# OpenRobotLab/EmbodiedScan

Measured on AMD Instinct MI355X. Metric: scans/sec (train step) mv-3ddet, 20x(480x640) RGB-D views, higher is better.
Workload: dtype bf16; 1 GPU; mv-3ddet ResNet-50(w16) + MinkResNet34 + FCAF3DHeadRotMat, 20 views 480x640, 100k points/scan, bf16 matrix cores with f32 accumulate / f32 master weights, full train step incl. H2D of the batch and AdamW; views=20, parallelism=dp1, h2d=157 MB per step as ONE copy from a pinned slab on a copy stream, double-buffered

## Files before the change

embodiedscan_amd/csrc/imgconv.hip:

```cpp
#include "common.h"
#include "../../include/es_hip.h"

typedef float f32x4 __attribute__((ext_vector_type(4)));
typedef __bf16 bf16x8_t __attribute__((ext_vector_type(8)));

__device__ __attribute__((aligned(16))) unsigned short g_ic_zero[8];

template <int C, int WP, int S, int MODE>
__global__ __launch_bounds__(256) void k_img_conv3(const void* __restrict__ Xv, int ldx, const unsigned short* __restrict__ Wt,
                                                   const float* __restrict__ scale, const float* __restrict__ shift,
                                                   const unsigned short* __restrict__ gate, int ldg, void* __restrict__ Yv, int ldy,
                                                   int y_half, int act, int H, int W, int rows_per_wg, int bands) {
  static_assert(MODE == 0 || S == 1, "the gated data gradient is built for stride 1");
  constexpr int RB = C * 2;
  constexpr int XP = S * WP + 2, X_BYTES = XP * RB;
  constexpr int NS = S == 1 ? 4 : 8;
  constexpr int GX = RB / 16;
  constexpr int NCB = C / 16;
  constexpr bool CO_SPLIT = NCB >= 4;
  constexpr int CBW = CO_SPLIT ? NCB / 4 : NCB;
  constexpr bool PAIR = C == 16;
  constexpr int KS = PAIR ? 1 : C / 32;
  constexpr int NT = PAIR ? 5 : 9;
  constexpr int NPB = WP / 16;
// ... 124 lines not shown
            }
          } else if (px < Wo) {
            const float gt = __uint_as_float((uint32_t)gate[row * ldg + col] << 16);
            ((float*)Yv)[row * ldy + col] = gt > 0.f ? v : 0.f;
          }
        }
      }
    }
  }
}

static int ES_OPT_IMG_CONV = 1;
static int ES_OPT_IMG_CONV_WGS = 1024;
extern "C" int es_img_conv_set_option(int key, int value) {
  if (key == 50) { ES_OPT_IMG_CONV = value; return 0; }
  if (key == 51) { ES_OPT_IMG_CONV_WGS = value; return 0; }
  return -1;
}

static bool img_conv_plan(int n_img, int H, int W, int C, int stride, int mode, int& wp, int& rows, int& bands) {
  if (!ES_OPT_IMG_CONV || n_img <= 0 || H <= 0 || W <= 0) return false;
  if (mode == 1 && stride != 1) return false;
  if (stride != 1 && !(stride == 2 && H % 2 == 0 && W % 2 == 0)) return false;
  const int Ho = H / stride, Wo = W / stride;
  if (C == 16 && Wo <= 128 && stride == 1) wp = Wo <= 64 ? 64 : 128;
  else if (C == 32 && Wo <= 64) wp = 64;
  else if (C == 64 && Wo <= 32) wp = 32;
  else return false;
  if (C == 64 && stride == 2) return false;
  const int target = (C == 64 || stride == 2) ? ES_OPT_IMG_CONV_WGS / 2 : ES_OPT_IMG_CONV_WGS;
  bands = target / n_img;
  if (bands < 1) bands = 1;
  if (bands > Ho) bands = Ho;
  rows = es_cdiv(Ho, bands);
  bands = es_cdiv(Ho, rows);
  return true;
}

static bool img_conv_check(int n_img, int H, int W, int C, int stride, int mode, const void* X, int ldx, const void* W_bf16,
                           const void* Y, int y_half, int ldy, int& wp, int& rows, int& bands) {
  if (!img_conv_plan(n_img, H, W, C, stride, mode, wp, rows, bands)) return false;
  if ((ldx % (mode ? 4 : 8)) || ((((uintptr_t)X) | ((uintptr_t)W_bf16)) & 15) || (y_half ? ((ldy % 2) || (((uintptr_t)Y) & 3)) : 0)) return false;
  if (mode == 1 && y_half) return false;
  return (long long)n_img * H * W * (ldx > ldy ? ldx : ldy) < (1ll << 31);
}

extern "C" int es_img_conv3_supported(int n_img, int H, int W, int C, int stride, int mode) {
  int wp, rows, bands;
  return img_conv_check(n_img, H, W, C, stride, mode, nullptr, C, nullptr, nullptr, 0, C, wp, rows, bands) ? 1 : 0;
}

extern "C" int es_img_conv3_bf16(const void* X, int ldx, const void* W_bf16, int n_img, int H, int W, int C, int stride, int mode,
                                 const float* scale, const float* shift, const void* gate, int ldg, int act, void* Y, int y_half,
                                 int ldy, void* stream) {
  int wp, rows, bands;
  if (!img_conv_check(n_img, H, W, C, stride, mode, X, ldx, W_bf16, Y, y_half, ldy, wp, rows, bands)) return -4;
  if (mode == 1 && gate == nullptr) return -4;
  if (mode == 0 && act != 0 && act != 1) return -4;
  hipStream_t st = (hipStream_t)stream;
  const unsigned short* Wt = (const unsigned short*)W_bf16;
  const unsigned short* G = (const unsigned short*)gate;
#define IC_LAUNCH(C_, WP_, S_, M_)                                                                                           \
  hipLaunchKernelGGL((k_img_conv3<C_, WP_, S_, M_>), dim3(n_img * bands), dim3(256), 0, st, X, ldx, Wt, scale, shift, G, ldg, Y, ldy, \
                     y_half, act, H, W, rows, bands)
  if (mode == 0 && stride == 1) {
    if (C == 16 && wp == 128) IC_LAUNCH(16, 128, 1, 0);
    else if (C == 16) IC_LAUNCH(16, 64, 1, 0);
    else if (C == 32) IC_LAUNCH(32, 64, 1, 0);
    else IC_LAUNCH(64, 32, 1, 0);
  } else if (mode == 0) {
    if (C == 32) IC_LAUNCH(32, 64, 2, 0);
    else if (C == 64) IC_LAUNCH(64, 32, 2, 0);
    else return -4;
  } else {
    if (C == 16 && wp == 128) IC_LAUNCH(16, 128, 1, 1);
    else if (C == 16) IC_LAUNCH(16, 64, 1, 1);
    else if (C == 32) IC_LAUNCH(32, 64, 1, 1);
    else IC_LAUNCH(64, 32, 1, 1);
  }
#undef IC_LAUNCH
  ES_CHECK_LAUNCH();
  return 0;
}
```

embodiedscan_amd/engine.py:

```python
import os

import torch
from . import hip
from .hip import P, call, iarr


def _stream():
    return hip.stream()


_NEW_VARS = None


class Var:
    __slots__ = ('d', 'g', 'rg', 'dh', 'gh', 'gate', 'gated', 'fresh')

    def __init__(self, d, rg=True):
        self.d, self.g, self.rg = d, None, rg
        self.dh = self.gh = None
        if _NEW_VARS is not None:
            _NEW_VARS.append(self)
        self.fresh = False
        self.gate = None
        self.gated = False
# ... 241 lines not shown
    ws['used'] = True
    _KEEP.extend(keep)
    return ws['h']


def wgrad_stream_obj():
    return _wgrad_rec()['s']


def join_wgrad_streams(final=True):
    cur = hip.stream_obj()
    for ws in _WGRAD_STREAMS.values():
        if ws['used']:
            ws['join'].record(ws['s'])
            cur.wait_event(ws['join'])
            ws['used'] = False
    if final:
        _KEEP.clear()


_ZEROED = ('ticket', 'split', 'colsum', 'topk')
_WS = {tag: {} for tag in ('wgrad', 'dense') + _ZEROED}
_WGRAD_WS = _WS['wgrad']


def stream_ws(stream, tag, floats, like):
    table = _WS[tag]
    ws = table.get(stream)
    if ws is None or ws.numel() < floats or ws.device != like.device:
        if ws is not None:
            _KEEP.append(ws)
        if tag in _ZEROED:
            ws = torch.zeros(max(int(floats), 1 << 16), dtype=torch.float32, device=like.device)
            if stream != _stream():
                ev = torch.cuda.Event()
                ev.record(hip.stream_obj())
                hip._stream_of(stream).wait_event(ev)
        else:
            ws = torch.empty(max(int(floats), 1 << 22), dtype=torch.float32, device=like.device)
        table[stream] = ws
    return ws, ws.numel()


def ticket_ws(floats, like, tag='ticket'):
    assert tag in _ZEROED, tag
    return stream_ws(_stream(), tag, floats, like)


GRAD_EPOCH = [1]
_GRAD_STAMP = {}


def new_grad_epoch():
    GRAD_EPOCH[0] += 1
    if len(_GRAD_STAMP) > 1 << 16:
        _GRAD_STAMP.clear()


def _first_write(ptr):
    acc = 1 if _GRAD_STAMP.get(ptr) == GRAD_EPOCH[0] else 0
    _GRAD_STAMP[ptr] = GRAD_EPOCH[0]
    return acc


def _written(ptr):
    return 1 if _GRAD_STAMP.get(ptr) == GRAD_EPOCH[0] else 0


def _wgrad(name, sw, dW, *args, like=None, acc=None):
    if name == 'es_spconv_wgrad_bf16_src':
        X, xh, ldx, dY, yh, ldy, nbr, n_out, n_in, K, cin, cout = args
        need = hip.raw('es_spconv_wgrad_workspace_floats')(1, X, xh, ldx, dY, yh, ldy, n_out, n_in, K, cin, cout)
    else:
        X, ldx, dY, ldy, nbr, n_out, n_in, K, cin, cout = args
        need = hip.raw('es_spconv_wgrad_workspace_floats')(int(name == 'es_spconv_wgrad_bf16'), X, 0, ldx, dY, 0, ldy, n_out, n_in,
                                                           K, cin, cout)
    if like is None:
        like = torch.empty(0, device=torch.device('cuda', torch.cuda.current_device()))
    ws, nf = stream_ws(sw, 'wgrad', need, like) if need else (None, 0)
    call(name, *args, dW, _first_write(dW) if acc is None else acc, P(ws), nf, sw)


IMG_WGRAD = [os.environ.get('ES_IMG_WGRAD', '1') != '0']
HEAD_BWD_FUSED = [os.environ.get('ES_HEAD_BWD_FUSED', '1') != '0']


GC_SETTLE_STEP = 6


_HOST_SETTLED = [False]


def settle_host_threads(force=False):
    if _HOST_SETTLED[0] and not force:
        return
    _HOST_SETTLED[0] = True
    want = os.environ.get('ES_HOST_THREADS', 'auto')
    if want == '0':
        return
    if want == 'auto':
        from .datasets.loader import effective_cpus
        local = max(1, int(os.environ.get('LOCAL_WORLD_SIZE', '1') or 1))
        n = max(1, effective_cpus() // 4 // local)
    else:
        n = max(1, int(want))
    if torch.get_num_threads() > n:
        torch.set_num_threads(n)


def settle_gc(det):
    settle_host_threads()
    n = getattr(det, '_steps_done', 0) + 1
    det._steps_done = n
    if n == GC_SETTLE_STEP and os.environ.get('ES_GC_FREEZE', '1') != '0':
        import gc
        gc.collect()
        gc.freeze()
        _GC_FROZEN[0] = True


def reset_tickets():
    for tag in _ZEROED:
        for ws in _WS[tag].values():
            ws[:min(ws.numel(), 2048)].zero_()


def drop_caches():
    for table in _WS.values():
        table.clear()
    _KEEP.clear()


MARKS = None


HOST_MARKS = None


def mark(name):
    if HOST_MARKS is not None:
        import time
        HOST_MARKS.append((name, time.perf_counter()))
    if MARKS is not None:
        ev = torch.cuda.Event(enable_timing=True)
        ev.record(hip.stream_obj())
        MARKS.append((name, ev))


DEBUG_GRADS = None
DEBUG_CONV = None
DEBUG_OPS = None
DEBUG_FWD = None


def fwd_record(kind, entry, **ops):
    rec = dict(kind=kind, entry=entry, precision=PRECISION[0])
    for k, v in ops.items():
        if isinstance(v, (Param, ParamSlice)):
            rec[k] = v.d.clone()
            if PRECISION[0] == 'bf16' and v.d.dim() == 3:
                rec[k + '_h'] = v.bf16()[1].clone()
        elif isinstance(v, torch.Tensor):
            rec[k] = v.clone()
        else:
            rec[k] = v
    if callable(DEBUG_FWD):
# ... 183 lines not shown
    x.fresh = False
    y.fresh = True
    return y


def _conv_backward(x, w, nbr, inv, n_out, y, gy, bias, bias_from, need_dx, bf, gate=None, dense=None, maps=None, img=None):
    K, cin, cout = w.d.shape
    rec = None
    dn_ok = bf and dense is not None and gate is None and _ld(gy) == cout and _ld(x.d) == cin
    dn_w = dense if (dn_ok and w.g is not None and dense_ok(dense, 2, cin, cout)) else None
    dn_d = dense if (dn_ok and need_dx and x.rg and dense_ok(dense, 1, cin, cout)) else None
    if maps is not None and (DEBUG_CONV is not None or (w.g is not None and dn_w is None) or (need_dx and x.rg and dn_d is None)):
        nbr, inv = maps.get()
    if DEBUG_CONV is not None:
        rec = dict(x=x.d, w=w, nbr=nbr, n_out=n_out, gy=gy.clone(), bf=bool(bf), gate=gate, need_dx=bool(need_dx and x.rg),
                   before=(x.g.clone() if (x.g is not None and need_dx and x.rg) else None), bias=bias, bias_from=bias_from)
        DEBUG_CONV.append(rec)
    gh = None
    if dn_w is not None or dn_d is not None or (
            bf and cout >= 16 and need_dx and x.rg and gate is None and _ld(gy) == cout and _use_shadow(n_out, cout, K, cout, cin)):
        gh = y.grad_shadow() if gy is y.g else _cast_rows(gy)
    if dn_w is not None:
        x.shadow()
    if w.g is not None or (bias is not None and bias.g is not None):
        sw = _wgrad_stream(gy, x.d, gh, x.dh)
    if w.g is not None:
        _conv_wgrad(x, w, nbr, n_out, gy, gh, bf, dn_w, maps, img, sw)
    if bias is not None and bias.g is not None:
        nb, dst = cout - bias_from, bias.g.data_ptr() + 4 * bias_from
        ws, nf = stream_ws(sw, 'colsum', int(hip.raw('es_colsum_workspace_floats')(n_out, nb)), gy)
        call('es_colsum', gy.data_ptr() + 4 * bias_from, _ld(gy), n_out, nb, dst, _first_write(dst), P(ws), nf, sw)
    if need_dx and x.rg:
        _conv_dgrad(x, w, inv, n_out, gy, gh, bf, dn_d, maps, gate, img)
    if rec is not None and rec['need_dx']:
        rec['after'] = x.g.clone()


def _conv_wgrad(x, w, nbr, n_out, gy, gh, bf, dn_w, maps, img, sw):
    K, cin, cout = w.d.shape
    n_in = x.d.shape[0]
    acc = _first_write(P(w.g))
    xh_f32 = bf and x.dh is not None and gy.dtype == torch.float32
    if dn_w is not None:
        if _dense_wgrad(P(x.dh), cin, P(gh), cout, dn_w, 0, cin, cout, P(w.g), acc, sw, gh):
            return
        if maps is not None:
            nbr, _ = maps.get()
            sw = _wgrad_stream()
    if IMG_WGRAD[0] and xh_f32 and img is not None and K == 9 and cin == cout:
        nf = int(hip.raw('es_img_wgrad9_workspace_floats')(img[0], img[1], img[2], cin, img[3]))
        if nf:
            ws, nf = stream_ws(sw, 'wgrad', nf, gy)
            if hip.try_call('es_img_wgrad9_bf16', P(x.dh), _ld(x.dh), P(gy), _ld(gy), img[0], img[1], img[2], cin, img[3], P(w.g), acc,
                            P(ws), nf, sw):
                return
    if xh_f32 and K == 1 and nbr is None and n_in == n_out:
        nf = int(hip.raw('es_rows_wgrad1_workspace_floats')(n_out, cin, cout))
        if nf:
            ws, nf = stream_ws(sw, 'wgrad', nf, gy)
            if hip.try_call('es_rows_wgrad1_bf16', P(x.dh), _ld(x.dh), P(gy), _ld(gy), n_out, cin, cout, P(w.g), acc, P(ws), nf, sw):
                return
    if bf and (gh is not None or x.dh is not None or x.d.dtype == torch.bfloat16):
        xs, ys = x.dh if x.dh is not None else x.d, gh if gh is not None else gy
        _wgrad('es_spconv_wgrad_bf16_src', sw, P(w.g), P(xs), int(x.dh is not None), _ld(xs), P(ys), int(gh is not None), _ld(ys),
               P(nbr), n_out, n_in, K, cin, cout, like=gy, acc=acc)
        return
    assert x.d.dtype == torch.float32, 'bf16 activation rows reach the weight gradient through their shadow (x.dh)'
    _wgrad('es_spconv_wgrad_bf16' if bf else 'es_spconv_wgrad', sw, P(w.g), P(x.d), _ld(x.d), P(gy), _ld(gy), P(nbr), n_out, n_in, K,
           cin, cout, like=gy, acc=acc)


def _conv_dgrad(x, w, inv, n_out, gy, gh, bf, dn_d, maps, gate, img):
    K, cin, cout = w.d.shape
    n_in = x.d.shape[0]
    s = _stream()
    if gate is not None:
        assert x.g is None and bf, 'gated dgrad: x must have exactly one consumer'
        x.g, x.gated = torch.empty(x.d.shape, dtype=torch.float32, device=x.d.device), True
        if (img is not None and K == 9 and img[3] == 1 and cin == cout and x.d.dtype == torch.bfloat16 and gy.dtype == torch.float32
                and _ld(x.d) == cin and hip.raw('es_img_conv3_supported')(img[0], img[1], img[2], cin, 1, 1) == 1
                and hip.try_call('es_img_conv3_bf16', P(gy), _ld(gy), P(w.bf16()[0]), img[0], img[1], img[2], cin, 1, 1, P(gate), 0, P(x.d),
                                 _ld(x.d), 3, P(x.g), 0, _ld(x.g), s)):
            return
        if x.d.dtype == torch.bfloat16:
            call('es_spconv_fwd_bf16_io', P(gy), 0, _ld(gy), P(w.bf16()[0]), P(inv), n_in, n_out, K, cout, cin, P(gate), 0,
                 P(x.d), 1, _ld(x.d), 3, P(x.g), 0, _ld(x.g), s)
        else:
            call('es_spconv_fwd_bf16_affine', P(gy), _ld(gy), P(w.bf16()[0]), P(inv), n_in, n_out, K, cout, cin, P(gate), 0,
                 P(x.d), _ld(x.d), 3, P(x.g), _ld(x.g), s)
        return
    g, acc = _grad_target(x, x.d)
    if dn_d is not None:
        if _dense_launch(P(gh), cout, P(w.bf16()[0]), dn_d, 1, cin, cout, P(g), _ld(g), acc, gh):
            return
        if maps is not None:
            _, inv = maps.get()
    if gh is not None and _halo_ok(inv, n_in, n_out, cout, K, cout, cin) and \
            _halo_launch(P(gh), cout, P(w.bf16()[0]), inv, n_in, n_out, K, cout, cin, 0, P(g), _ld(g), acc):
        return
    if gh is not None:
        _fwd_bf16(P(gh), 1, cout, P(w.bf16()[0]), P(inv), n_in, n_out, K, cout, cin, 0, P(g), _ld(g), acc, gh)
    elif bf and cout >= 16:
        _fwd_bf16(P(gy), 0, _ld(gy), P(w.bf16()[0]), P(inv), n_in, n_out, K, cout, cin, 0, P(g), _ld(g), acc, gy)
    else:
        call('es_spconv_fwd', P(gy), _ld(gy), P(w.d), P(inv), n_in, n_out, K, cout, cin, 0, P(g), _ld(g), 1, acc, s)


def conv_affine(x, w, nbr, inv, n_out, scale, shift, act=1, res=None, need_dx=True, sole_consumer=False, out_bf16=False, img=None):
    K, cin, cout = w.d.shape
    n_in = x.d.shape[0]
    if PRECISION[0] != 'bf16':
        return affine_act(conv(x, w, nbr, inv, n_out, need_dx=need_dx), scale, shift, act=act, res=res)
    h16 = torch.bfloat16
    y16 = bool(out_bf16 and cout % 4 == 0)
    x16, r16 = x.d.dtype == h16, (res is not None and res.d.dtype == h16)
    y = Var(empty((n_out, cout), x.d, dtype=h16 if y16 else torch.float32))
    ic = (img is not None and K == 9 and x16 and res is None and act in (0, 1) and cin == cout and _ld(x.d) == cin
          and hip.raw('es_img_conv3_supported')(img[0], img[1], img[2], cin, img[3], 0) == 1)
    if ic and hip.try_call('es_img_conv3_bf16', P(x.d), cin, P(w.bf16()[1]), img[0], img[1], img[2], cin, img[3], 0, P(scale), P(shift), 0,
                           0, act, P(y.d), int(y16), cout, _stream()):
        entry = 'es_img_conv3_bf16'
    elif x16 or r16 or y16:
        call('es_spconv_fwd_bf16_io', P(x.d), int(x16), _ld(x.d), P(w.bf16()[1]), P(nbr), n_out, n_in, K, cin, cout, P(scale),
             P(shift), P(res.d) if res is not None else 0, int(r16), _ld(res.d) if res is not None else 0, act, P(y.d),
             int(y16), cout, _stream())
        entry = 'es_spconv_fwd_bf16_io'
    else:
        call('es_spconv_fwd_bf16_affine', P(x.d), _ld(x.d), P(w.bf16()[1]), P(nbr), n_out, n_in, K, cin, cout, P(scale),
             P(shift), P(res.d) if res is not None else 0, _ld(res.d) if res is not None else 0, act, P(y.d), cout, _stream())
        entry = 'es_spconv_fwd_bf16_affine'
    if y16:
        y.dh = y.d
    if x16:
        x.dh = x.d
    if DEBUG_FWD is not None:
        fwd_record('conv_affine', entry, x=x.d, w=w, nbr=nbr, n_out=n_out, round=True, scale=scale, shift=shift,
                   res=res.d if res is not None else None, act=act, y=y.d)

    if act == 1 and res is None:
        y.gate = scale
    gate = x.gate if sole_consumer else None

    def bwd():
        if y.g is None:
            return
        if DEBUG_GRADS is not None:
            DEBUG_GRADS[id(y)] = y.g.clone()
        if y.gated:
            gconv = y.g
        else:
            gr = accr = 0
            if res is not None and res.rg:
                t, accr = _grad_target(res, res.d)
                gr = P(t)
            gconv = torch.empty((n_out, cout), dtype=torch.float32, device=y.d.device)
            call('es_affine_act_bwd_yh' if y.d.dtype == h16 else 'es_affine_act_bwd', P(y.g), P(y.d), P(scale), n_out, cout, act,
                 P(gconv), 0, gr, accr, _stream())
        _conv_backward(x, w, nbr, inv, n_out, y, gconv, None, 0, need_dx, True, gate, img=img)
    TAPE.add(bwd)
    return y


def gen_conv_transpose(x, w):
    K, cin, cout = w.d.shape
    n = x.d.shape[0]
    y = Var(empty((n * 8, cout), x.d))
    s = _stream()
    bf = PRECISION[0] == 'bf16'
    fused = False
    if bf and GEN_FUSED[0] and x.d.dtype == torch.float32:
        fused = hip.raw('es_gen_transpose_fwd_bf16')(P(x.d), _ld(x.d), P(w.bf16()[1]), n, cin, cout, P(y.d), s) == 0
    for k in range(0 if not fused else 8, 8):
        if bf:
            call('es_spconv_fwd_bf16', P(x.d), 0, _ld(x.d), w.bf16()[1].data_ptr() + 2 * k * cin * cout, 0, n, n, 1, cin,
# ... 502 lines not shown
```

embodiedscan_amd/models/backbones/resnet2d.py:

```python
import os
import torch
from ... import engine as E
from ... import hip
from ...hip import P, call
from ...registry import MODELS

STEM_POOL = [os.environ.get('ES_STEM_POOL', '1') != '0']


def _stream():
    return hip.stream()


class _Grid:

    def __init__(self, n_img, H, W, dev):
        self.n_img, self.H, self.W, self.dev = n_img, H, W, dev
        self.maps = {}

    def conv_map(self, kh, stride, pad, want_inv=True):
        key = (kh, stride, pad)
        if key not in self.maps:
            Ho, Wo = (self.H + 2 * pad - kh) // stride + 1, (self.W + 2 * pad - kh) // stride + 1
            n_out, K = self.n_img * Ho * Wo, kh * kh
# ... 57 lines not shown

    def forward(self, x):
        n_img, H, W, _ = x.shape
        dev = x.device
        a16 = bool(self.act16 and E.PRECISION[0] == 'bf16' and self.frozen_stages >= 0)
        fused = self.base in (16, 32, 64) and self.frozen_stages >= 0 and a16 and STEM_POOL[0]
        direct = (self.base in (16, 32) and self.frozen_stages >= 0) or fused
        key = (n_img, H, W, direct)
        if key not in self.grids:
            if direct:
                Ho, Wo = (H + 6 - 7) // 2 + 1, (W + 6 - 7) // 2 + 1
                stem, nbr_a, nbr_b = (None, None, n_img * Ho * Wo, Ho, Wo), None, None
            else:
                stem = _Grid(n_img, H, W, dev).conv_map(7, 2, 3, want_inv=False)
                nbr_a, nbr_b = stem[0][:, :27].contiguous(), stem[0][:, 27:].contiguous()
            g1 = _Grid(n_img, stem[3], stem[4], dev)
            pool = g1.conv_map(3, 2, 1, want_inv=False)
            grids = [_Grid(n_img, pool[3], pool[4], dev)]
            for li in range(1, 4):
                h, w = grids[-1].H, grids[-1].W
                grids.append(_Grid(n_img, (h + 2 - 3) // 2 + 1, (w + 2 - 3) // 2 + 1, dev))
            self.grids[key] = (stem, nbr_a, nbr_b, pool, grids)
        stem, nbr_a, nbr_b, pool, grids = self.grids[key]
        s = _stream()
        prev = E.TAPE.enabled
        E.TAPE.enabled = prev and self.frozen_stages < 0
        w1 = self.arena.p[self.prefix + 'conv1.weight']
        xin = x.reshape(n_img * H * W, 3)
        if fused:
            yp = torch.empty((pool[2], self.base), dtype=torch.bfloat16, device=dev)
            call('es_stem_pool_fwd', P(xin), P(w1), P(self.fold['bn1'][0]), P(self.fold['bn1'][1]), n_img, H, W, self.base, P(yp), s)
            if E.DEBUG_FWD is not None:
                E.fwd_record('stem', 'es_stem_pool_fwd', x=xin, w=w1, scale=self.fold['bn1'][0], shift=self.fold['bn1'][1], n_img=n_img,
                             H=H, W=W, pooled=True, y=yp)
            cur = None
        elif self.base in (16, 32) and self.frozen_stages >= 0:
            y = torch.empty((stem[2], self.base), dtype=torch.float32, device=dev)
            call('es_stem_conv_fwd', P(xin), P(w1), P(self.fold['bn1'][0]), P(self.fold['bn1'][1]), n_img, H, W,
                 self.base, P(y), s)
            if E.DEBUG_FWD is not None:
                E.fwd_record('stem', 'es_stem_conv_fwd', x=xin, w=w1, scale=self.fold['bn1'][0], shift=self.fold['bn1'][1], n_img=n_img,
                             H=H, W=W, pooled=False, y=y)
            cur = E.Var(y, rg=False)
        else:
            y = torch.empty((stem[2], self.base), dtype=torch.float32, device=dev)
            call('es_spconv_fwd', P(xin), 3, P(w1), P(nbr_a), stem[2], xin.shape[0], 27, 3, self.base, 0, P(y),
                 self.base, 0, 0, s)
            call('es_spconv_fwd', P(xin), 3, w1.data_ptr() + 4 * 27 * 3 * self.base, P(nbr_b), stem[2], xin.shape[0], 22,
                 3, self.base, 0, P(y), self.base, 0, 1, s)
            cur = E.affine_act(E.Var(y, rg=False), *self.fold['bn1'], act=1)
        if cur is None:
            cur = E.Var(yp, rg=False)
            cur.dh = yp
        elif a16:
            yp = torch.empty((pool[2], self.base), dtype=torch.bfloat16, device=dev)
            call('es_maxpool_fwd_h', P(cur.d), self.base, P(pool[0]), pool[2], pool[0].shape[1], self.base, P(yp), s)
            if E.DEBUG_FWD is not None:
                E.fwd_record('maxpool', 'es_maxpool_fwd_h', x=cur.d, nbr=pool[0], y=yp, arg=None)
            cur = E.Var(yp, rg=False)
            cur.dh = yp
        else:
            cur = E.maxpool(cur, pool[0], pool[2], need_dx=False)
        cur.rg = self.frozen_stages < 0
        outs = []
        for li, nblk in enumerate(self.arch[50]):
            E.TAPE.enabled = prev and (li + 1) > self.frozen_stages
            gin = grids[li - 1] if li > 0 else grids[0]
            for bi in range(nblk):
                p = f'layer{li + 1}.{bi}.'
                stride = 2 if (bi == 0 and li > 0) else 1
                g_in = gin if bi == 0 else grids[li]
                o = E.conv_affine(cur, self._par(p + 'conv1.weight'), None, None, cur.d.shape[0], *self.fold[p + 'bn1'],
                                  act=1, out_bf16=a16)
                nbr, inv, n_out, _, _ = g_in.conv_map(3, stride, 1)
                o = E.conv_affine(o, self._par(p + 'conv2.weight'), nbr, inv, n_out, *self.fold[p + 'bn2'], act=1,
                                  sole_consumer=True, out_bf16=a16, img=(n_img, g_in.H, g_in.W, stride))
                if bi == 0:
                    if stride == 1:
                        idt = E.conv_affine(cur, self._par(p + 'downsample.0.weight'), None, None, n_out,
                                            *self.fold[p + 'downsample.1'], act=0, out_bf16=a16)
                    else:
                        dn, di, _, _, _ = g_in.conv_map(1, stride, 0)
                        idt = E.conv_affine(cur, self._par(p + 'downsample.0.weight'), dn, di, n_out,
                                            *self.fold[p + 'downsample.1'], act=0, out_bf16=a16)
                else:
                    idt = cur
                cur = E.conv_affine(o, self._par(p + 'conv3.weight'), None, None, n_out, *self.fold[p + 'bn3'], act=1,
                                    res=idt, sole_consumer=True, out_bf16=a16)
                if not E.TAPE.enabled:
                    cur.rg = False
            if li in self.out_indices:
                outs.append((cur, grids[li].H, grids[li].W))
        E.TAPE.enabled = prev
        return outs

    def __call__(self, x):
        E.refresh_weight_copies()
        key = (x.data_ptr(), tuple(x.shape), E.PRECISION[0], bool(self.act16), E.TAPE.enabled, self._fold_version,
               self.arena.data.data_ptr())
        return E.graphed(self._graphs, key, lambda: self.forward(x))
```

include/es_hip.h:

```cpp
#ifndef ES_HIP_H
#define ES_HIP_H
#include <stddef.h>
#include <stdint.h>
#ifdef __cplusplus
extern "C" {
#endif

#define ES_MAX_SEG 32

#define ES_MAX_BATCH 512
int es_voxel_keys(const float* points, int n, int ld, int batch, float voxel_size, int64_t* keys, void* stream);
int es_unique_first(const int64_t* keys, int n, int64_t* tkeys, int* tvals, int cap, int* scratch,
                    int64_t* out_keys, int* out_src, int* count_host, void* stream);
size_t es_sort_scratch_bytes(int n);
int es_morton_sort(const int64_t* keys, const int* src, int n, void* scratch, size_t scratch_bytes, int64_t* out_keys,
                   int* out_src, void* stream);
int es_sort_u64(const int64_t* keys, const int* src, int n, void* scratch, size_t scratch_bytes, int64_t* out_keys, int* out_src,
                void* stream);
int es_draw_keys(const float* depth, int V, int HW, size_t seed, float* values, int64_t* keys, void* stream);
int es_draw_keys_index(int n, size_t seed, int stream_id, float* values, int64_t* keys, void* stream);
int es_draw_unpack(const int64_t* keys, int n, const int* in_view, const int* in_pix, int* out_view, int* out_pix, void* stream);
int es_build_table(const int64_t* keys, int n, int64_t* tkeys, int* tvals, int cap, void* stream);
int es_stride_keys(const int64_t* in_keys, int n, int out_ts, int64_t* out_keys, void* stream);
int es_keys_to_coords(const int64_t* keys, int n, int* coords , void* stream);
// ... 206 lines not shown
int es_layernorm_fwd(const float* x, const float* res, int n, int C, const float* w, const float* b, float eps, float* y,
                     float* z, float* mean, float* rstd, void* stream);
size_t es_layernorm_bwd_workspace_floats(int n, int C);
int es_layernorm_bwd(const float* dy, const float* z, int n, int C, const float* w, const float* mean, const float* rstd,
                     float* dz, int accumulate, float* dw, float* db, float* workspace, size_t workspace_floats, void* stream);
int es_text_embed_ln(const long long* ids, int B, int T, int pad_id, const float* word, const float* pos, const float* type0,
                     int C, int vocab, int max_pos, const float* ln_w, const float* ln_b, float eps, float* y, int* pos_ids,
                     void* stream);
int es_text_add_ln(const float* x, const float* res, int n, int C, const float* w, const float* b, float eps, float* y,
                   void* stream);
int es_bias_gelu(float* x, int ld, int n, int C, const float* bias, void* stream);
int es_text_attn_fwd(const float* qkv, int ld, int B, int H, int T, const int* mask_dev, float* O, int ldo, int bf16,
                     void* stream);
int es_relu_fwd(float* x, size_t n, void* stream);
int es_relu_bwd(float* dy, const float* y, size_t n, void* stream);
int es_contrastive_fwd(const float* v, int B, int L, const float* text, int T, int C, const int* tlen_dev, const int* vlen_dev,
                       const float* bias_dev, float* logits, int Tout, float* rowmax, void* stream);
int es_contrastive_shared_fwd(const float* v, int L, const float* text, int P, int T, int C, const int* tlen_dev,
                              const float* bias_dev, float* logits, int Tout, float* rowmax, void* stream);
size_t es_contrastive_bwd_workspace_floats(int B, int T);
int es_contrastive_bwd(const float* dlogits, int Tout, const float* v, int B, int L, const float* text, int T, int C,
                       const int* tlen_dev, float* dv, int acc_v, float* dtext , float* dbias , float* workspace,
                       size_t workspace_floats, void* stream);
int es_ground_decode_fwd(const float* pred, int ldp, const float* points, int n, float* box , void* stream);
int es_ground_decode_bwd(const float* pred, int ldp, const float* dbox, int n, float* dpred, int ldg, int accumulate,
                         void* stream);
int es_ground_decode_fcaf_fwd(const float* pred, int ldp, const float* points, int n, float* box , void* stream);
int es_ground_decode_fcaf_bwd(const float* pred, int ldp, const float* dbox, int n, float* dpred, int ldg, int accumulate,
                              void* stream);
int es_box3d_iou(const float* boxes1, int N, const float* boxes2, int M, float* iou, void* stream);
#define ES_DET_MAX_THR 8
int es_det_best_gt(const float* pred_boxes, int P, const int* pred_grp, const float* gt_boxes, const int* grp_off_dev, int n_grp,
                   float* iou_max, int* gt_best, void* stream);
int es_det_mark(const float* iou_max, const int* gt_best, const int* order, int P, const float* thr_host, int T, int G, int* claim,
                unsigned char* tp, void* stream);
int es_det_ap(const unsigned char* tp, int P, const int* cls_off_dev, const int* npos_dev, int C, int T, float* ap, int* tp_total,
              void* stream);
int es_ground_hits(const float* boxes, const int* box_off_dev, const int* topk_idx, int S, int K, const float* gt_boxes,
                   const int* gt_off_dev, const float* thr_host, int T, int* hit, float* iou_top, void* stream);
int es_ground_tally(const int* hit, const unsigned char* flags, int N, int T, int* counts, void* stream);
int es_occ_confusion(const long long* pred, const int* gt, int n, int C, int* counts, void* stream);
int es_ground_match(const float* logits, int Tout, const float* boxes, int B, int Q, const float* gt_boxes,
                    const unsigned char* pos_map, const int* gt_off_dev, int Gmax, const int* tlen_dev, int T, float w_cls,
                    float w_l1, float w_iou, double* cost, double* work, int* iwork, int* q2g, void* stream);
int es_ground_focal(const float* logits, int Tout, int B, int Q, const int* q2g, const unsigned char* pos_map,
                    const int* gt_off_dev, const int* tlen_dev, int T, float alpha, float gamma, const float* avg_factor_dev,
                    float grad_scale, float* dlogits, double* loss_sum, void* stream);
int es_box_cd_pairs(const float* pred, const int* q2g, int B, int Q, const float* gt_boxes, const int* gt_off_dev, int n_pairs,
                    float grad_scale, const float* group_w_host, float* dpred, double* loss_acc, void* stream);
int es_topk_sorted(const float* vals, int B, int L, const int* vlen_dev, int k, int* idx, void* stream);

int es_dconv_supported(const int* geom_host, int mode, int Cin, int Cout);
size_t es_dconv_workspace_floats(const int* geom_host, int mode, int Cin, int Cout);
int es_dconv_fwd_bf16(const void* Xh, int ldx, const void* W_bf16, const int* geom_host, int mode, int Cin, int Cout, float* Y,
                      int ldy, int accumulate, float* ws, size_t ws_floats, void* stream);
int es_dconv_wgrad_bf16(const void* Xh, int ldx, const void* dYh, int ldy, const int* geom_host, int transposed, int Cin, int Cout,
                        float* dW, int accumulate, void* stream);
size_t es_dconv_wgrad_workspace_floats(const int* geom_host, int transposed, int Cin, int Cout);
int es_dconv_wgrad_ws_bf16(const void* Xh, int ldx, const void* dYh, int ldy, const int* geom_host, int transposed, int Cin, int Cout,
                           float* dW, int accumulate, float* ws, size_t ws_floats, void* stream);
int es_dconv_set_option(int key, int value);

size_t es_halo_plan_rows(int n_out);
int es_halo_plan(const int* nbr, int n_out, int K, void* loc, int* hrows, int* hcnt, void* stream);
int es_halo_set_option(int key, int value);
int es_spconv_halo_supported(int n_out, int n_in, int ldx, int K, int Cin, int Cout);
int es_spconv_halo_bf16(const void* Xh, int ldx, const void* W_bf16, const void* loc, const int* hrows, const int* hcnt, int n_out,
                        int n_in, int K, int Cin, int Cout, const float* bias, float* Y, int ldy, int accumulate, int mirror, void* stream);

size_t es_img_wgrad9_workspace_floats(int n_img, int H, int W, int C, int stride);
int es_img_wgrad9_bf16(const void* Xh, int ldx, const float* dY, int ldy, int n_img, int H, int W, int C, int stride, float* dW,
                       int accumulate, float* ws, size_t ws_floats, void* stream);
int es_img_wgrad_set_option(int key, int value);
size_t es_rows_wgrad1_workspace_floats(int n, int Cin, int Cout);
int es_rows_wgrad1_bf16(const void* Xh, int ldx, const float* dY, int ldy, int n, int Cin, int Cout, float* dW, int accumulate, float* ws,
                        size_t ws_floats, void* stream);

int es_img_conv3_supported(int n_img, int H, int W, int C, int stride, int mode);
int es_img_conv3_bf16(const void* X, int ldx, const void* W_bf16, int n_img, int H, int W, int C, int stride, int mode,
                      const float* scale, const float* shift, const void* gate, int ldg, int act, void* Y, int y_half, int ldy,
                      void* stream);
int es_img_conv_set_option(int key, int value);

#ifdef __cplusplus
}
#endif
#endif
```

Before: 175.2 scans/s.

## Add dense stride-2 image dgrad kernels for 3x3 and 1x1 ResNet convs

Adds two HIP kernels for the data gradient of stride-2 convolutions in the 2D ResNet backbone. The first handles the gated 3x3 case by splitting output pixels into four parity classes, staging output-gradient rows in a shared-memory ring and running MFMA against preloaded weights. The second handles the 1x1 downsample case as a tiled GEMM that scatters into the strided input positions and zero-fills the others. Both replace the generic sparse-conv path, which gathers through neighbor index maps, with direct dense-grid addressing. The cost is extra specialised code with shape limits (even H and W, C of 32 or 64, alignment checks); anything outside those limits falls back to the old path.

```diff
diff --git a/embodiedscan_amd/csrc/imgconv.hip b/embodiedscan_amd/csrc/imgconv.hip
--- a/embodiedscan_amd/csrc/imgconv.hip
+++ b/embodiedscan_amd/csrc/imgconv.hip
@@ -230,3 +230,288 @@
   ES_CHECK_LAUNCH();
   return 0;
 }
+
+template <int C, int WPO>
+__global__ __launch_bounds__(256) void k_img_dgrad3_s2(const float* __restrict__ G, int ldg, const unsigned short* __restrict__ Wn,
+                                                       const float* __restrict__ scale, const unsigned short* __restrict__ gate, int lda,
+                                                       float* __restrict__ dX, int ldx, int H, int W, int cells_per_wg, int bands) {
+  constexpr int RB = C * 2;
+  constexpr int XP = WPO + 1, X_BYTES = XP * RB;
+  constexpr int NS = 4;
+  constexpr int NCB = C / 16;
+  constexpr bool CO_SPLIT = NCB >= 4;
+  constexpr int CBW = CO_SPLIT ? NCB / 4 : NCB;
+  constexpr int KS = C / 32;
+  constexpr int NPB = WPO / 16;
+  __shared__ __attribute__((aligned(16))) unsigned char smem[NS * X_BYTES];
+  const int t = threadIdx.x, lane = t & 63, wv = t >> 6, li = lane & 15, kq = lane >> 4;
+  const int im = blockIdx.x / bands, band = blockIdx.x - im * bands;
+  const int Ho = H / 2, Wo = W / 2;
+  const int c0 = band * cells_per_wg, c1 = min(Ho, c0 + cells_per_wg);
+  if (c0 >= c1) return;
+  for (int i = t; i < NS * X_BYTES / 16; i += 256) ((uint4*)smem)[i] = make_uint4(0u, 0u, 0u, 0u);
+
+  bf16x8_t Bf[9][KS][CBW];
+#pragma unroll
+  for (int k = 0; k < 9; ++k)
+#pragma unroll
+    for (int ks = 0; ks < KS; ++ks)
+#pragma unroll
+      for (int cw = 0; cw < CBW; ++cw) {
+        const int cb = CO_SPLIT ? wv * CBW + cw : cw;
+        const uint4 v = *(const uint4*)(Wn + ((size_t)k * C + cb * 16 + li) * C + ks * 32 + kq * 8);
+        Bf[k][ks][cw] = __builtin_bit_cast(bf16x8_t, v);
+      }
+  __syncthreads();
+
+  constexpr int NLG = (WPO * C / 4 + 255) / 256;
+  float4 greg[NLG];
+  auto load_g = [&](int oy) {
+    const float* src = G + ((size_t)im * Ho + oy) * Wo * ldg;
+#pragma unroll
+    for (int j = 0; j < NLG; ++j) {
+      const int e = j * 256 + t, px = e / (C / 4), c4 = e - px * (C / 4);
+      greg[j] = (oy < Ho && px < Wo) ? *(const float4*)(src + (size_t)px * ldg + c4 * 4) : make_float4(0.f, 0.f, 0.f, 0.f);
+    }
+  };
+  auto store_g = [&](int oy) {
+    if (oy >= Ho) return;
+    unsigned char* dst = smem + (oy & (NS - 1)) * X_BYTES;
+#pragma unroll
+    for (int j = 0; j < NLG; ++j) {
+      const int e = j * 256 + t, px = e / (C / 4), c4 = e - px * (C / 4);
+      if (px < WPO) {
+        uint2 v;
+        v.x = es_pack_bf16(greg[j].x, greg[j].y);
+        v.y = es_pack_bf16(greg[j].z, greg[j].w);
+        *(uint2*)(dst + px * RB + c4 * 8) = v;
+      }
+    }
+  };
+
+  load_g(c0);
+  store_g(c0);
+  load_g(c0 + 1);
+  for (int cy = c0; cy < c1; ++cy) {
+    store_g(cy + 1);
+    __syncthreads();
+    load_g(cy + 2);
+#pragma unroll 1
+    for (int pb = CO_SPLIT ? 0 : wv; pb < NPB; pb += CO_SPLIT ? 1 : 4) {
+      const int q0 = pb * 16;
+      if (q0 >= Wo) break;
+#pragma unroll
+      for (int cls = 0; cls < 4; ++cls) {
+        const int yr = cls >> 1, px = cls & 1;
+        f32x4 acc[CBW];
+#pragma unroll
+        for (int cw = 0; cw < CBW; ++cw) acc[cw] = (f32x4){0.f, 0.f, 0.f, 0.f};
+#pragma unroll
+        for (int ky = 0; ky < 3; ++ky) {
+          if ((ky == 1) != (yr == 0)) continue;
+          const int oy = (yr == 1 && ky == 0) ? cy + 1 : cy;
+          const bool rowok = oy < Ho;
+#pragma unroll
+          for (int kx = 0; kx < 3; ++kx) {
+            if ((kx == 1) != (px == 0)) continue;
+            const int k = ky * 3 + kx;
+            const int ox = q0 + li + ((px == 1 && kx == 0) ? 1 : 0);
+            const unsigned char* xr = smem + (oy & (NS - 1)) * X_BYTES + ox * RB;
+#pragma unroll
+            for (int ks = 0; ks < KS; ++ks) {
+              uint4 av = *(const uint4*)(xr + (ks * 32 + kq * 8) * 2);
+              if (!rowok) av = make_uint4(0u, 0u, 0u, 0u);
+              const bf16x8_t a = __builtin_bit_cast(bf16x8_t, av);
+#pragma unroll
+              for (int cw = 0; cw < CBW; ++cw) acc[cw] = __builtin_amdgcn_mfma_f32_16x16x32_bf16(a, Bf[k][ks][cw], acc[cw], 0, 0, 0);
+            }
+          }
+        }
+        const size_t rowy = ((size_t)im * H + 2 * cy + yr) * W;
+#pragma unroll
+        for (int cw = 0; cw < CBW; ++cw) {
+          const int col = (CO_SPLIT ? wv * CBW + cw : cw) * 16 + li;
+          const float sc = scale ? scale[col] : 1.f;
+#pragma unroll
+          for (int r = 0; r < 4; ++r) {
+            const int q = q0 + kq * 4 + r;
+            if (q < Wo) {
+              const size_t row = rowy + 2 * q + px;
+              const float v = (acc[cw][r] + 0.f) * sc + 0.f;
+              const float gt = __uint_as_float((uint32_t)gate[row * lda + col] << 16);
+              dX[row * ldx + col] = gt > 0.f ? v : 0.f;
+            }
+          }
+        }
+      }
+    }
+  }
+}
+
+#define ES_S2_LD 48
+template <int NT>
+__global__ __launch_bounds__(256) void k_img_dgrad1_s2(const float* __restrict__ G, int ldg, const unsigned short* __restrict__ Wn, int n_g,
+                                                       int Kred, int Wo, float* __restrict__ dX, int ldx, int accumulate) {
+  constexpr int NF = NT / 16;
+  constexpr int NB = (NT + 63) / 64;
+  constexpr int LD = ES_S2_LD;
+  __shared__ __attribute__((aligned(16))) unsigned short As[2 * 128 * LD];
+  __shared__ __attribute__((aligned(16))) unsigned short Bs[2 * NT * LD];
+  const int t = threadIdx.x, lane = t & 63, wv = t >> 6, li = lane & 15, kq = lane >> 4;
+  const int row0 = blockIdx.x * 128, n0 = blockIdx.y * NT;
+  if (!accumulate) {
+    constexpr int C4 = NT / 4;
+    const float4 z = make_float4(0.f, 0.f, 0.f, 0.f);
+    for (int e = t; e < 128 * C4; e += 256) {
+      const int r = e / C4, c4 = e - r * C4, row = row0 + r;
+      if (row < n_g) {
+        const int q = row / Wo, ox = row - q * Wo;
+        float* p = dX + ((size_t)4 * q * Wo + 2 * ox) * ldx + n0 + c4 * 4;
+        *(float4*)(p + ldx) = z;
+        *(float4*)(p + (size_t)2 * Wo * ldx) = z;
+        *(float4*)(p + ((size_t)2 * Wo + 1) * ldx) = z;
+      }
+    }
+  }
+  f32x4 acc[2][NF];
+#pragma unroll
+  for (int a = 0; a < 2; ++a)
+#pragma unroll
+    for (int b = 0; b < NF; ++b) acc[a][b] = (f32x4){0.f, 0.f, 0.f, 0.f};
+  const int nC = Kred / 32;
+  const int a_r = t >> 1, a_kk = (t & 1) * 16;
+  const int b_n = t >> 2, b_kk = (t & 3) * 8;
+  const int b_w = ((NT % 64 == 0) || b_n < NT) ? b_n : 0;
+  const bool a_ok = row0 + a_r < n_g;
+  const float* a_src = G + (size_t)(a_ok ? row0 + a_r : 0) * ldg + a_kk;
+  struct Regs { float4 a[4]; uint4 b[NB]; };
+  auto load_chunk = [&](Regs& R, int c) {
+    const float4* pa = (const float4*)(a_src + c * 32);
+#pragma unroll
+    for (int q = 0; q < 4; ++q) R.a[q] = pa[q];
+#pragma unroll
+    for (int h = 0; h < NB; ++h) R.b[h] = *(const uint4*)(Wn + (size_t)(n0 + b_w + h * 64) * Kred + c * 32 + b_kk);
+  };
+  auto store_chunk = [&](const Regs& R, int buf) {
+    uint4 v0 = make_uint4(es_pack_bf16(R.a[0].x, R.a[0].y), es_pack_bf16(R.a[0].z, R.a[0].w), es_pack_bf16(R.a[1].x, R.a[1].y),
+                          es_pack_bf16(R.a[1].z, R.a[1].w));
+    uint4 v1 = make_uint4(es_pack_bf16(R.a[2].x, R.a[2].y), es_pack_bf16(R.a[2].z, R.a[2].w), es_pack_bf16(R.a[3].x, R.a[3].y),
+                          es_pack_bf16(R.a[3].z, R.a[3].w));
+    if (!a_ok) v0 = v1 = make_uint4(0u, 0u, 0u, 0u);
+    uint4* pa = (uint4*)&As[buf * 128 * LD + a_r * LD + a_kk];
+    pa[0] = v0;
+    pa[1] = v1;
+#pragma unroll
+    for (int h = 0; h < NB; ++h)
+      if ((NT % 64 == 0) || b_n < NT) *(uint4*)&Bs[buf * NT * LD + (b_n + h * 64) * LD + b_kk] = R.b[h];
+  };
+  auto compute = [&](int buf) {
+    bf16x8_t a[2], b[NF];
+#pragma unroll
+    for (int mf = 0; mf < 2; ++mf) a[mf] = *(const bf16x8_t*)&As[buf * 128 * LD + (wv * 32 + mf * 16 + li) * LD + kq * 8];
+#pragma unroll
+    for (int nf = 0; nf < NF; ++nf) b[nf] = *(const bf16x8_t*)&Bs[buf * NT * LD + (nf * 16 + li) * LD + kq * 8];
+#pragma unroll
+    for (int mf = 0; mf < 2; ++mf)
+#pragma unroll
+      for (int nf = 0; nf < NF; ++nf) acc[mf][nf] = __builtin_amdgcn_mfma_f32_16x16x32_bf16(a[mf], b[nf], acc[mf][nf], 0, 0, 0);
+  };
+  Regs R;
+  load_chunk(R, 0);
+  store_chunk(R, 0);
+  load_chunk(R, nC > 1 ? 1 : 0);
+  __syncthreads();
+  for (int c = 0; c < nC; ++c) {
+    if (c + 1 < nC) store_chunk(R, (c + 1) & 1);
+    load_chunk(R, c + 2 < nC ? c + 2 : c);
+    compute(c & 1);
+    __syncthreads();
+  }
+#pragma unroll
+  for (int mf = 0; mf < 2; ++mf)
+#pragma unroll
+    for (int nf = 0; nf < NF; ++nf)
+#pragma unroll
+      for (int r = 0; r < 4; ++r) {
+        const int row = row0 + wv * 32 + mf * 16 + kq * 4 + r;
+        if (row < n_g) {
+          const int q = row / Wo, ox = row - q * Wo;
+          float* p = dX + ((size_t)4 * q * Wo + 2 * ox) * ldx + n0 + nf * 16 + li;
+          const float v = acc[mf][nf][r] + 0.f;
+          *p = accumulate ? (*p + v) : v;
+        }
+      }
+}
+
+static int ES_OPT_IMG_S2 = 1;
+static int ES_OPT_IMG_S2_WGS = 2048;
+extern "C" int es_img_stride_set_option(int key, int value) {
+  if (key == 52) { ES_OPT_IMG_S2 = value; return 0; }
+  if (key == 53) { ES_OPT_IMG_S2_WGS = value; return 0; }
+  return -1;
+}
+
+static bool img_dgrad3_s2_check(int n_img, int H, int W, int C, const void* G, int ldg, const void* Wn, const void* gate, int lda,
+                                const void* dX, int ldx, int& cells, int& bands) {
+  if (!ES_OPT_IMG_S2 || n_img <= 0 || H <= 0 || W <= 0 || (H % 2) || (W % 2)) return false;
+  const int Ho = H / 2, Wo = W / 2;
+  if (!((C == 32 && Wo <= 64) || (C == 64 && Wo <= 32))) return false;
+  if ((ldg % 4) || (ldx % 4) || ldg < C || ldx < C || lda < C) return false;
+  if ((((uintptr_t)G) | ((uintptr_t)Wn) | ((uintptr_t)dX)) & 15) return false;
+  const int ldm = ldx > lda ? ldx : lda;
+  if ((long long)n_img * H * W * ldm >= (1ll << 31) || (long long)n_img * Ho * Wo * ldg >= (1ll << 31)) return false;
+  bands = ES_OPT_IMG_S2_WGS / n_img;
+  if (bands < 1) bands = 1;
+  if (bands > Ho) bands = Ho;
+  cells = es_cdiv(Ho, bands);
+  bands = es_cdiv(Ho, cells);
+  return true;
+}
+
+extern "C" int es_img_dgrad3_s2_supported(int n_img, int H, int W, int C) {
+  int cells, bands;
+  return img_dgrad3_s2_check(n_img, H, W, C, nullptr, C, nullptr, nullptr, C, nullptr, C, cells, bands) ? 1 : 0;
+}
+
+extern "C" int es_img_dgrad3_s2_bf16(const float* G, int ldg, const void* Wn_bf16, int n_img, int H, int W, int C, const float* scale,
+                                     const void* gate, int lda, float* dX, int ldx, void* stream) {
+  int cells, bands;
+  if (!img_dgrad3_s2_check(n_img, H, W, C, G, ldg, Wn_bf16, gate, lda, dX, ldx, cells, bands)) return -4;
+  if (G == nullptr || Wn_bf16 == nullptr || gate == nullptr || dX == nullptr) return -4;
+  hipStream_t st = (hipStream_t)stream;
+  const unsigned short* Wn = (const unsigned short*)Wn_bf16;
+  const unsigned short* A = (const unsigned short*)gate;
+  if (C == 32)
+    hipLaunchKernelGGL((k_img_dgrad3_s2<32, 64>), dim3(n_img * bands), dim3(256), 0, st, G, ldg, Wn, scale, A, lda, dX, ldx, H, W, cells, bands);
+  else
+    hipLaunchKernelGGL((k_img_dgrad3_s2<64, 32>), dim3(n_img * bands), dim3(256), 0, st, G, ldg, Wn, scale, A, lda, dX, ldx, H, W, cells, bands);
+  ES_CHECK_LAUNCH();
+  return 0;
+}
+
+static bool img_dgrad1_s2_check(int n_img, int H, int W, int Cg, int Cx, const void* G, int ldg, const void* Wn, const void* dX, int ldx) {
+  if (!ES_OPT_IMG_S2 || n_img <= 0 || H <= 0 || W <= 0 || (H % 2) || (W % 2)) return false;
+  if (Cg <= 0 || Cx <= 0 || (Cg % 32) || (Cx % 32)) return false;
+  if ((ldg % 4) || (ldx % 4) || ldg < Cg || ldx < Cx) return false;
+  if ((((uintptr_t)G) | ((uintptr_t)Wn) | ((uintptr_t)dX)) & 15) return false;
+  return (long long)n_img * H * W * ldx < (1ll << 31) && (long long)n_img * (H / 2) * (W / 2) * ldg < (1ll << 31);
+}
+
+extern "C" int es_img_dgrad1_s2_supported(int n_img, int H, int W, int Cg, int Cx) {
+  return img_dgrad1_s2_check(n_img, H, W, Cg, Cx, nullptr, Cg, nullptr, nullptr, Cx) ? 1 : 0;
+}
+
+extern "C" int es_img_dgrad1_s2_bf16(const float* G, int ldg, const void* Wn_bf16, int n_img, int H, int W, int Cg, int Cx, float* dX, int ldx,
+                                     int accumulate, void* stream) {
+  if (!img_dgrad1_s2_check(n_img, H, W, Cg, Cx, G, ldg, Wn_bf16, dX, ldx)) return -4;
+  if (G == nullptr || Wn_bf16 == nullptr || dX == nullptr) return -4;
+  hipStream_t st = (hipStream_t)stream;
+  const unsigned short* Wn = (const unsigned short*)Wn_bf16;
+  const int n_g = n_img * (H / 2) * (W / 2), Wo = W / 2;
+  if (Cx % 128 == 0)
+    hipLaunchKernelGGL((k_img_dgrad1_s2<128>), dim3(es_cdiv(n_g, 128), Cx / 128), dim3(256), 0, st, G, ldg, Wn, n_g, Cg, Wo, dX, ldx, accumulate);
+  else
+    hipLaunchKernelGGL((k_img_dgrad1_s2<32>), dim3(es_cdiv(n_g, 128), Cx / 32), dim3(256), 0, st, G, ldg, Wn, n_g, Cg, Wo, dX, ldx, accumulate);
+  ES_CHECK_LAUNCH();
+  return 0;
+}
diff --git a/embodiedscan_amd/engine.py b/embodiedscan_amd/engine.py
--- a/embodiedscan_amd/engine.py
+++ b/embodiedscan_amd/engine.py
@@ -347,6 +347,7 @@
 
 
 IMG_WGRAD = [os.environ.get('ES_IMG_WGRAD', '1') != '0']
+IMG_STRIDED_DGRAD = [os.environ.get('ES_IMG_STRIDED_DGRAD', '1') != '0']
 HEAD_BWD_FUSED = [os.environ.get('ES_HEAD_BWD_FUSED', '1') != '0']
 
 
@@ -696,6 +697,11 @@
                 and hip.try_call('es_img_conv3_bf16', P(gy), _ld(gy), P(w.bf16()[0]), img[0], img[1], img[2], cin, 1, 1, P(gate), 0, P(x.d),
                                  _ld(x.d), 3, P(x.g), 0, _ld(x.g), s)):
             return
+        if (IMG_STRIDED_DGRAD[0] and img is not None and K == 9 and img[3] == 2 and cin == cout and x.d.dtype == torch.bfloat16
+                and gy.dtype == torch.float32 and hip.raw('es_img_dgrad3_s2_supported')(img[0], img[1], img[2], cin) == 1
+                and hip.try_call('es_img_dgrad3_s2_bf16', P(gy), _ld(gy), P(w.bf16()[0]), img[0], img[1], img[2], cin, P(gate), P(x.d),
+                                 _ld(x.d), P(x.g), _ld(x.g), s)):
+            return
         if x.d.dtype == torch.bfloat16:
             call('es_spconv_fwd_bf16_io', P(gy), 0, _ld(gy), P(w.bf16()[0]), P(inv), n_in, n_out, K, cout, cin, P(gate), 0,
                  P(x.d), 1, _ld(x.d), 3, P(x.g), 0, _ld(x.g), s)
@@ -704,6 +710,11 @@
                  P(x.d), _ld(x.d), 3, P(x.g), _ld(x.g), s)
         return
     g, acc = _grad_target(x, x.d)
+    if (IMG_STRIDED_DGRAD[0] and img is not None and K == 1 and img[3] == 2 and bf and gh is None and dn_d is None
+            and gy.dtype == torch.float32 and g.dtype == torch.float32 and n_in == img[0] * img[1] * img[2]
+            and hip.raw('es_img_dgrad1_s2_supported')(img[0], img[1], img[2], cout, cin) == 1
+            and hip.try_call('es_img_dgrad1_s2_bf16', P(gy), _ld(gy), P(w.bf16()[0]), img[0], img[1], img[2], cout, cin, P(g), _ld(g), acc, s)):
+        return
     if dn_d is not None:
         if _dense_launch(P(gh), cout, P(w.bf16()[0]), dn_d, 1, cin, cout, P(g), _ld(g), acc, gh):
             return
diff --git a/embodiedscan_amd/models/backbones/resnet2d.py b/embodiedscan_amd/models/backbones/resnet2d.py
--- a/embodiedscan_amd/models/backbones/resnet2d.py
+++ b/embodiedscan_amd/models/backbones/resnet2d.py
@@ -163,7 +163,7 @@
                     else:
                         dn, di, _, _, _ = g_in.conv_map(1, stride, 0)
                         idt = E.conv_affine(cur, self._par(p + 'downsample.0.weight'), dn, di, n_out,
-                                            *self.fold[p + 'downsample.1'], act=0, out_bf16=a16)
+                                            *self.fold[p + 'downsample.1'], act=0, out_bf16=a16, img=(n_img, g_in.H, g_in.W, stride))
                 else:
                     idt = cur
                 cur = E.conv_affine(o, self._par(p + 'conv3.weight'), None, None, n_out, *self.fold[p + 'bn3'], act=1,
diff --git a/include/es_hip.h b/include/es_hip.h
--- a/include/es_hip.h
+++ b/include/es_hip.h
@@ -312,6 +312,14 @@
                       void* stream);
 int es_img_conv_set_option(int key, int value);
 
+int es_img_dgrad3_s2_supported(int n_img, int H, int W, int C);
+int es_img_dgrad3_s2_bf16(const float* G, int ldg, const void* Wn_bf16, int n_img, int H, int W, int C, const float* scale,
+                          const void* gate, int lda, float* dX, int ldx, void* stream);
+int es_img_dgrad1_s2_supported(int n_img, int H, int W, int Cg, int Cx);
+int es_img_dgrad1_s2_bf16(const float* G, int ldg, const void* Wn_bf16, int n_img, int H, int W, int Cg, int Cx, float* dX, int ldx,
+                          int accumulate, void* stream);
+int es_img_stride_set_option(int key, int value);
+
 #ifdef __cplusplus
 }
 #endif
```

Measured after the change: 177.9 scans/s, median of 6. +1.5%, better.
